# OSU-Nowlab/MPI4DL

Hardware: NVIDIA H100
Metric: images/sec (device-timed, max over ranks) AmoebaNet-D 8192^2 hot path (spatial-stage conv/pool fwd+bwd) (higher is better)
Workload: dtype bf16

## Files before the change

### include/spconv.h

```cpp
#ifndef SPCONV_H_
#define SPCONV_H_

#include <stddef.h>
#include <stdint.h>

#ifdef __cplusplus
extern "C" {
#endif

#define SPC_VERSION 101

enum { SPC_OK = 0, SPC_EINVAL = -1, SPC_ECUDA = -2, SPC_EUNSUPPORTED = -3, SPC_ENOMEM = -4 };
enum { SPC_F32 = 0, SPC_BF16 = 1 };
enum { SPC_POOL_MAX = 0, SPC_POOL_AVG = 1 };
enum {
  SPC_ALGO_AUTO = 0, SPC_ALGO_DIRECT = 1, SPC_ALGO_TCGEN05 = 2, SPC_ALGO_TF32 = 3, SPC_ALGO_TF32_ALL = 4,
  SPC_ALGO_TF32_STRIDED = 5
};

typedef struct {
  int32_t N, C, H, W;
  int32_t K, R, S;
  int32_t stride_h, stride_w;
  int32_t pad_h, pad_w;
// ... 11 lines not shown
typedef struct {
  const void* strip[9];
} spc_halo;

int         spc_version(void);
const char* spc_last_error(void);
int         spc_device_info(int device, int* sm_count, int* cc);
long long   spc_launch_count(int reset);
void        spc_reload_env(void);

int spc_conv2d_fwd(const spc_conv_desc* d, const void* x, const spc_halo* halo, const void* w,
                   const void* bias, void* y, void* workspace, size_t workspace_bytes,
                   void* stream);

int spc_conv2d_fwd_interior(const spc_conv_desc* d, const void* x, const void* w, const void* bias,
                            void* y, void* workspace, size_t workspace_bytes, void* stream);
int spc_conv2d_fwd_boundary(const spc_conv_desc* d, const void* x, const spc_halo* halo,
                            const void* w, const void* bias, void* y, void* stream);

int spc_conv2d_dgrad(const spc_conv_desc* d, const void* dy, const void* w, void* dx,
                     void* workspace, size_t workspace_bytes, void* stream);

int spc_conv2d_wgrad(const spc_conv_desc* d, const void* x, const spc_halo* halo, const void* dy,
                     float* dw, float* db, int accumulate, void* workspace,
                     size_t workspace_bytes, void* stream);

size_t spc_conv_workspace_bytes(const spc_conv_desc* d, int op );
int    spc_conv_uses_tcgen05(const spc_conv_desc* d, int op);
void   spc_conv_out_shape(const spc_conv_desc* d, int* Ho, int* Wo);

int spc_pool2d_fwd(const spc_pool_desc* d, const void* x, const spc_halo* halo, void* y, void* stream);
int spc_pool2d_bwd(const spc_pool_desc* d, const void* x, const spc_halo* halo, const void* dy,
                   void* dx, void* stream);

size_t spc_bn_workspace_bytes(int N, int C, long long HW);
int spc_bn_stats(int N, int C, long long HW, int dtype, const void* y, float* mean, float* var, void* workspace,
                 size_t workspace_bytes, void* stream);
int spc_bn_apply(int N, int C, long long HW, int dtype, const void* y, const float* mean, const float* rstd,
                 const float* gamma, const float* beta, int relu, void* z, void* stream);
int spc_bn_bwd_reduce(int N, int C, long long HW, int dtype, const void* dz, const void* y, const float* mean,
                      const float* rstd, const float* gamma, const float* beta, int relu, float* dsum,
                      float* dsumx, void* workspace, size_t workspace_bytes, void* stream);
int spc_bn_bwd_apply(int N, int C, long long HW, int dtype, const void* dz, const void* y, const float* mean,
                     const float* rstd, const float* gamma, const float* beta, int relu, const float* dsum,
                     const float* dsumx, void* dy, void* stream);

int spc_halo_pack(int N, int C, int H, int W, int halo_h, int halo_w, int dtype, const void* x,
                  void* const send[9], void* stream);
int spc_halo_pad(int N, int C, int H, int W, int halo_h, int halo_w, int dtype, const void* x,
                 const spc_halo* halo, void* y, void* stream);
int spc_halo_crop(int N, int C, int H, int W, int halo_h, int halo_w, int dtype, const void* dy,
                  void* dx, void* stream);

typedef struct spc_mailbox spc_mailbox;
#define SPC_IPC_HANDLE_BYTES 64
int   spc_mailbox_create(spc_mailbox** out, size_t bytes, int nflags);
void  spc_mailbox_destroy(spc_mailbox* mb);
void* spc_mailbox_data(spc_mailbox* mb);
int   spc_mailbox_export(spc_mailbox* mb, unsigned char handle[SPC_IPC_HANDLE_BYTES]);
int   spc_mailbox_open(spc_mailbox** out, const unsigned char handle[SPC_IPC_HANDLE_BYTES],
                       size_t bytes, int nflags);
int spc_halo_post(int N, int C, int H, int W, int halo_h, int halo_w, int dtype, const void* x,
                  void* const send[9], spc_mailbox* self, spc_mailbox* const peers[9],
                  const int ack_idx[9], uint32_t ack_seq, const int arrival_idx[9], uint32_t seq,
                  void* stream);
int spc_halo_collect(void* const dst[9], const void* const src[9], const size_t bytes[9],
// ... 29 lines not shown
```

### mpi4dl_b200/_lib.py

```python
import ctypes as C
import os

HERE = os.path.dirname(os.path.abspath(__file__))
LIB_PATH = os.path.join(HERE, "libspconv.so")

SPC_F32, SPC_BF16 = 0, 1
SPC_POOL_MAX, SPC_POOL_AVG = 0, 1
SPC_ALGO_AUTO, SPC_ALGO_DIRECT, SPC_ALGO_TCGEN05, SPC_ALGO_TF32, SPC_ALGO_TF32_ALL, SPC_ALGO_TF32_STRIDED = 0, 1, 2, 3, 4, 5
IPC_HANDLE_BYTES = 64


class ConvDesc(C.Structure):
    _fields_ = [(n, C.c_int32) for n in
                ("N", "C", "H", "W", "K", "R", "S", "stride_h", "stride_w", "pad_h", "pad_w", "dtype", "algo")]


class PoolDesc(C.Structure):
    _fields_ = [(n, C.c_int32) for n in ("N", "C", "H", "W", "k", "stride", "pad", "mode", "dtype")]


class Halo(C.Structure):
    _fields_ = [("strip", C.c_void_p * 9)]


_P = C.c_void_p
SYMBOLS = [
    ("spc_version", C.c_int, []),
    ("spc_last_error", C.c_char_p, []),
    ("spc_device_info", C.c_int, [C.c_int, C.POINTER(C.c_int), C.POINTER(C.c_int)]),
    ("spc_launch_count", C.c_longlong, [C.c_int]),
    ("spc_reload_env", None, []),
    ("spc_conv2d_fwd", C.c_int, [C.POINTER(ConvDesc), _P, C.POINTER(Halo), _P, _P, _P, _P, C.c_size_t, _P]),
    ("spc_conv2d_fwd_interior", C.c_int, [C.POINTER(ConvDesc), _P, _P, _P, _P, _P, C.c_size_t, _P]),
    ("spc_conv2d_fwd_boundary", C.c_int, [C.POINTER(ConvDesc), _P, C.POINTER(Halo), _P, _P, _P, _P]),
    ("spc_conv2d_dgrad", C.c_int, [C.POINTER(ConvDesc), _P, _P, _P, _P, C.c_size_t, _P]),
    ("spc_conv2d_wgrad", C.c_int, [C.POINTER(ConvDesc), _P, C.POINTER(Halo), _P, _P, _P, C.c_int, _P, C.c_size_t, _P]),
    ("spc_conv_workspace_bytes", C.c_size_t, [C.POINTER(ConvDesc), C.c_int]),
    ("spc_conv_uses_tcgen05", C.c_int, [C.POINTER(ConvDesc), C.c_int]),
    ("spc_conv_out_shape", None, [C.POINTER(ConvDesc), C.POINTER(C.c_int), C.POINTER(C.c_int)]),
    ("spc_pool2d_fwd", C.c_int, [C.POINTER(PoolDesc), _P, C.POINTER(Halo), _P, _P]),
    ("spc_pool2d_bwd", C.c_int, [C.POINTER(PoolDesc), _P, C.POINTER(Halo), _P, _P, _P]),
    ("spc_bn_workspace_bytes", C.c_size_t, [C.c_int, C.c_int, C.c_longlong]),
    ("spc_bn_stats", C.c_int, [C.c_int, C.c_int, C.c_longlong, C.c_int, _P, _P, _P, _P, C.c_size_t, _P]),
    ("spc_bn_apply", C.c_int, [C.c_int, C.c_int, C.c_longlong, C.c_int, _P, _P, _P, _P, _P, C.c_int, _P, _P]),
    ("spc_bn_bwd_reduce", C.c_int, [C.c_int, C.c_int, C.c_longlong, C.c_int, _P, _P, _P, _P, _P, _P, C.c_int, _P, _P, _P,
                                    C.c_size_t, _P]),
    ("spc_bn_bwd_apply", C.c_int, [C.c_int, C.c_int, C.c_longlong, C.c_int, _P, _P, _P, _P, _P, _P, C.c_int, _P, _P, _P, _P]),
    ("spc_halo_pack", C.c_int, [C.c_int] * 7 + [_P, C.POINTER(_P * 9), _P]),
    ("spc_halo_pad", C.c_int, [C.c_int] * 7 + [_P, C.POINTER(Halo), _P, _P]),
    ("spc_halo_crop", C.c_int, [C.c_int] * 7 + [_P, _P, _P]),
    ("spc_mailbox_create", C.c_int, [C.POINTER(_P), C.c_size_t, C.c_int]),
    ("spc_mailbox_destroy", None, [_P]),
    ("spc_mailbox_data", _P, [_P]),
    ("spc_mailbox_export", C.c_int, [_P, C.c_char_p]),
    ("spc_mailbox_open", C.c_int, [C.POINTER(_P), C.c_char_p, C.c_size_t, C.c_int]),
    ("spc_halo_post", C.c_int, [C.c_int] * 7 + [_P, C.POINTER(_P * 9), _P, C.POINTER(_P * 9), C.POINTER(C.c_int * 9),
                                C.c_uint32, C.POINTER(C.c_int * 9), C.c_uint32, _P]),
    ("spc_halo_collect", C.c_int, [C.POINTER(_P * 9), C.POINTER(_P * 9), C.POINTER(C.c_size_t * 9), _P, C.POINTER(_P * 9),
                                   C.POINTER(C.c_int * 9), C.c_uint32, C.POINTER(C.c_int * 9), _P]),
    ("spc_halo_post_auto", C.c_int, [C.c_int] * 7 + [_P, C.POINTER(_P * 9), C.c_size_t, _P, C.POINTER(_P * 9),
                                     C.POINTER(C.c_int * 9), C.POINTER(C.c_int * 9), C.c_int, C.c_int, _P]),
    ("spc_halo_collect_auto", C.c_int, [C.POINTER(_P * 9), C.POINTER(_P * 9), C.POINTER(C.c_size_t * 9), C.c_size_t, _P,
                                        C.POINTER(_P * 9), C.POINTER(C.c_int * 9), C.POINTER(C.c_int * 9), C.c_int, C.c_int,
                                        _P]),
    ("spc_conv2d_dgrad_halo", C.c_int, [C.POINTER(ConvDesc), _P, _P, C.POINTER(_P * 9), _P]),
    ("spc_pool2d_bwd_halo", C.c_int, [C.POINTER(PoolDesc), _P, C.POINTER(Halo), _P, C.POINTER(_P * 9), _P]),
    ("spc_halo_ring", C.c_int, [C.c_int] * 7 + [_P, C.POINTER(_P * 9), _P]),
    ("spc_halo_accumulate", C.c_int, [C.c_int] * 7 + [_P, C.POINTER(_P * 9), _P]),
    ("spc_halo_post_strips_auto", C.c_int, [C.POINTER(_P * 9), C.POINTER(C.c_size_t * 9), C.POINTER(_P * 9), C.c_size_t,
                                            _P, C.POINTER(_P * 9), C.POINTER(C.c_int * 9), C.POINTER(C.c_int * 9),
                                            C.c_int, C.c_int, _P]),
    ("spc_mailbox_signal", C.c_int, [_P, C.c_int, C.c_uint32, _P]),
    ("spc_mailbox_wait", C.c_int, [_P, C.c_int, C.c_uint32, _P]),
]
# ... 46 lines not shown
```

### mpi4dl_b200/build.py

```python
import os
import subprocess
import sys

HERE = os.path.dirname(os.path.abspath(__file__))
CSRC = os.path.join(HERE, "csrc")
LIB = os.path.join(HERE, "libspconv.so")
SOURCES = ["api.cu", "conv_direct.cu", "pool.cu", "halo.cu", "gemm_tc.cu", "conv_tap.cu", "wgrad_tap.cu", "bnrelu.cu",
           "halo_grad.cu", "gemm_tf32.cu", "conv_tap_tf32.cu", "conv_tap_s2_tf32.cu",
           "gemm_px.cu"]
NVCC_FLAGS = [
    "-O3", "-std=c++17", "-gencode", "arch=compute_90a,code=sm_90a", "-lineinfo",
    "-Xcompiler", "-fPIC", "--expt-relaxed-constexpr",
]


def _stale(target, deps):
    if not os.path.exists(target):
        return True
    t = os.path.getmtime(target)
    return any(os.path.getmtime(d) > t for d in deps)


def build_lib(force=False, verbose=False):
    nvcc = os.environ.get("NVCC", "/usr/local/cuda/bin/nvcc")
    hdrs = [os.path.join(CSRC, f) for f in os.listdir(CSRC) if f.endswith((".cuh", ".h"))]
    hdrs.append(os.path.join(HERE, "..", "include", "spconv.h"))
    objs = []
    procs = []
    for s in SOURCES:
        src = os.path.join(CSRC, s)
        obj = os.path.join(CSRC, s.replace(".cu", ".o"))
        objs.append(obj)
        if force or _stale(obj, [src] + hdrs):
            cmd = [nvcc] + NVCC_FLAGS + (["-Xptxas", "-v"] if verbose else []) + ["-c", src, "-o", obj]
            procs.append((s, subprocess.Popen(cmd, stdout=subprocess.PIPE, stderr=subprocess.STDOUT, text=True)))
    for s, p in procs:
        out, _ = p.communicate()
        if p.returncode != 0:
            sys.stderr.write(out)
            raise RuntimeError("nvcc failed on %s" % s)
        if verbose:
            sys.stderr.write(out)
# ... 9 lines not shown
```

### mpi4dl_b200/csrc/common.cuh

```cuda
#pragma once
#include <cuda_bf16.h>
#include <cuda_runtime.h>
#include <stdint.h>
#include <stdio.h>

#include "../../include/spconv.h"

namespace spc {

void set_error(const char* fmt, ...);
void count_launch(int n = 1);

#define SPC_CHECK_CUDA(expr)                                                              \
  do {                                                                                    \
    cudaError_t _e = (expr);                                                              \
    if (_e != cudaSuccess) {                                                              \
      spc::set_error("%s:%d CUDA error %s: %s", __FILE__, __LINE__, #expr,                \
                     cudaGetErrorString(_e));                                             \
      return SPC_ECUDA;                                                                   \
    }                                                                                     \
  } while (0)

#define SPC_REQUIRE(cond, ...)                                                            \
  do {                                                                                    \
    if (!(cond)) {                                                                        \
      spc::set_error(__VA_ARGS__);                                                        \
      return SPC_EINVAL;                                                                  \
    }                                                                                     \
  } while (0)

template <typename T> __device__ __forceinline__ float to_f32(T v);
template <> __device__ __forceinline__ float to_f32<float>(float v) { return v; }
template <> __device__ __forceinline__ float to_f32<__nv_bfloat16>(__nv_bfloat16 v) { return __bfloat162float(v); }
template <typename T> __device__ __forceinline__ T from_f32(float v);
template <> __device__ __forceinline__ float from_f32<float>(float v) { return v; }
template <> __device__ __forceinline__ __nv_bfloat16 from_f32<__nv_bfloat16>(float v) { return __float2bfloat16_rn(v); }

__device__ __forceinline__ bool pool_max_takes(float v, float m) { return (v > m) | (v != v); }
__device__ __forceinline__ float pool_max(float m, float v) {
  float r;
  asm("max.NaN.f32 %0, %1, %2;" : "=f"(r) : "f"(m), "f"(v));
  return r;
}

struct TileView {
  const void* x;
  const void* strip[9];
  int N, C, H, W;
  int hh, hw;
};

template <typename T>
__device__ __forceinline__ float tile_load(const TileView& v, int n, int c, int h, int w) {
  const bool hin = (unsigned)h < (unsigned)v.H;
  const bool win = (unsigned)w < (unsigned)v.W;
  if (hin && win) {
    if (v.x == nullptr) return 0.f;
    return to_f32<T>(reinterpret_cast<const T*>(v.x)[(((size_t)n * v.C + c) * v.H + h) * v.W + w]);
  }
  const int dr = h < 0 ? 0 : (hin ? 1 : 2);
  const int dc = w < 0 ? 0 : (win ? 1 : 2);
  const T* s = reinterpret_cast<const T*>(v.strip[dr * 3 + dc]);
  if (s == nullptr) return 0.f;
  const int sh = (dr == 1) ? v.H : v.hh;
  const int sw = (dc == 1) ? v.W : v.hw;
  const int y = (dr == 0) ? h + v.hh : (dr == 2 ? h - v.H : h);
  const int xx = (dc == 0) ? w + v.hw : (dc == 2 ? w - v.W : w);
  if ((unsigned)y >= (unsigned)sh || (unsigned)xx >= (unsigned)sw) return 0.f;
  return to_f32<T>(s[(((size_t)n * v.C + c) * sh + y) * sw + xx]);
}

template <typename T>
__device__ __forceinline__ const T* tile_ptr(const TileView& v, int n, int c, int h, int w) {
  const bool hin = (unsigned)h < (unsigned)v.H;
  const bool win = (unsigned)w < (unsigned)v.W;
// ... 104 lines not shown
```

### mpi4dl_b200/csrc/gemm_tc.cu

```cuda
#include <stdlib.h>

#include "common.cuh"
#include "tc_common.cuh"

namespace spc {

using namespace tc;

bool tap_v2_supported(int M, int Cin, int R, int S, int H, int W, int N, int stride);
int run_conv_tap_v2(const __nv_bfloat16* wp, int Mpad, int Cpad, const __nv_bfloat16* x, const __nv_bfloat16* bias,
                    __nv_bfloat16* y, int M, int Cin, int R, int S, int ph, int H, int W, int N, cudaStream_t st);

bool wgrad_tap_supported(int K, int C, int R, int S, int H, int W, int stride);
int run_wgrad_tap(const __nv_bfloat16* x, const __nv_bfloat16* dy, float* dw, int K, int C, int N, int H, int W, int R, int S,
                  cudaStream_t st);

int run_pw_px(int NT, const CUtensorMap& tw, const CUtensorMap& tx, const CUtensorMap& ty, int M, int Cin, int N, int P,
              int x5, int y5, const __nv_bfloat16* bias, int sms, cudaStream_t st);

namespace {

constexpr int TC_THREADS = 384;
constexpr int BK = 64;
constexpr int A_BLK_BYTES = 128 * BK * 2;
// ... 806 lines not shown
    const __nv_bfloat16* t0 = t + ((n * 4 + 2 * a) * C + c) * plane + (size_t)oy * Wo + v * 8;
    const uint4 e = __ldg(reinterpret_cast<const uint4*>(t0));
    const uint4 o = __ldg(reinterpret_cast<const uint4*>(t0 + (size_t)C * plane));
    uint4 lo, hi;
    lo.x = __byte_perm(e.x, o.x, 0x5410); lo.y = __byte_perm(e.x, o.x, 0x7632);
    lo.z = __byte_perm(e.y, o.y, 0x5410); lo.w = __byte_perm(e.y, o.y, 0x7632);
    hi.x = __byte_perm(e.z, o.z, 0x5410); hi.y = __byte_perm(e.z, o.z, 0x7632);
    hi.z = __byte_perm(e.w, o.w, 0x5410); hi.w = __byte_perm(e.w, o.w, 0x7632);
    uint4* d = reinterpret_cast<uint4*>(dx + ((nc * 2 * Ho) + 2 * oy + a) * (size_t)(2 * Wo) + v * 16);
    d[0] = lo; d[1] = hi;
  }
}

__global__ void subsample2_kernel(const __nv_bfloat16* __restrict__ x, __nv_bfloat16* __restrict__ y, size_t planes,
                                  int H, int W) {
  const int Ho = H / 2, Wo = W / 2, wv = Wo / 8;
  const size_t total = planes * Ho * wv;
  for (size_t i = (size_t)blockIdx.x * blockDim.x + threadIdx.x; i < total; i += (size_t)gridDim.x * blockDim.x) {
    const int v = (int)(i % wv);
    const int oy = (int)((i / wv) % Ho);
    const size_t pl = i / ((size_t)wv * Ho);
    const uint4* src = reinterpret_cast<const uint4*>(x + (pl * H + 2 * oy) * W + v * 16);
    const uint4 a = __ldg(src), b = __ldg(src + 1);
    uint4 o;
    o.x = __byte_perm(a.x, a.y, 0x5410);
    o.y = __byte_perm(a.z, a.w, 0x5410);
    o.z = __byte_perm(b.x, b.y, 0x5410);
    o.w = __byte_perm(b.z, b.w, 0x5410);
    *reinterpret_cast<uint4*>(y + (pl * Ho + oy) * Wo + v * 8) = o;
  }
}
__global__ void upsample2_zero_kernel(const __nv_bfloat16* __restrict__ g, __nv_bfloat16* __restrict__ dx,
                                      size_t planes, int H, int W) {
  const int Ho = H / 2, Wo = W / 2, wv = Wo / 8;
  const size_t total = planes * Ho * wv;
  const uint4 z = make_uint4(0, 0, 0, 0);
  for (size_t i = (size_t)blockIdx.x * blockDim.x + threadIdx.x; i < total; i += (size_t)gridDim.x * blockDim.x) {
    const int v = (int)(i % wv);
    const int oy = (int)((i / wv) % Ho);
    const size_t pl = i / ((size_t)wv * Ho);
    const uint4 a = __ldg(reinterpret_cast<const uint4*>(g + (pl * Ho + oy) * Wo + v * 8));
    uint4 lo, hi;
    lo.x = a.x & 0xFFFFu; lo.y = a.x >> 16; lo.z = a.y & 0xFFFFu; lo.w = a.y >> 16;
    hi.x = a.z & 0xFFFFu; hi.y = a.z >> 16; hi.z = a.w & 0xFFFFu; hi.w = a.w >> 16;
    uint4* d0 = reinterpret_cast<uint4*>(dx + (pl * H + 2 * oy) * W + v * 16);
    uint4* d1 = reinterpret_cast<uint4*>(dx + (pl * H + 2 * oy + 1) * W + v * 16);
    d0[0] = lo; d0[1] = hi; d1[0] = z; d1[1] = z;
  }
}
int launch_resample(bool up, const void* src, void* dst, size_t planes, int H, int W, cudaStream_t st) {
  const size_t total = planes * (H / 2) * (W / 16);
  size_t blocks = (total + 255) / 256;
  if (blocks > 132 * 32) blocks = 132 * 32;
  if (up)
    upsample2_zero_kernel<<<(int)blocks, 256, 0, st>>>((const __nv_bfloat16*)src, (__nv_bfloat16*)dst, planes, H, W);
  else
    subsample2_kernel<<<(int)blocks, 256, 0, st>>>((const __nv_bfloat16*)src, (__nv_bfloat16*)dst, planes, H, W);
  count_launch();
  SPC_CHECK_CUDA(cudaGetLastError());
  return SPC_OK;
}

__global__ void shift_copies_kernel(const __nv_bfloat16* __restrict__ x, __nv_bfloat16* __restrict__ xs,
                                    size_t planes, int H, int W, int S, int pw, int cs) {
  const int Wv = W / cs;
  const int wv = Wv / 8;
  const size_t rows = planes * H;
  const size_t total = rows * wv * S;
  for (size_t i = (size_t)blockIdx.x * blockDim.x + threadIdx.x; i < total; i += (size_t)gridDim.x * blockDim.x) {
    const int v = (int)(i % wv);
    const size_t row = (i / wv) % rows;
    const int sidx = (int)(i / ((size_t)wv * rows));
    const __nv_bfloat16* src = x + row * W;
    const int w0 = v * 8 * cs + sidx - pw;
    __nv_bfloat16 e[8];
#pragma unroll
    for (int j = 0; j < 8; ++j) {
      const int w = w0 + j * cs;
      e[j] = ((unsigned)w < (unsigned)W) ? src[w] : __float2bfloat16(0.f);
    }
    *reinterpret_cast<uint4*>(xs + ((size_t)sidx * rows + row) * Wv + v * 8) = *reinterpret_cast<const uint4*>(e);
  }
}
template <int S, int PW>
// ... 298 lines not shown
```

### mpi4dl_b200/csrc/pool.cu

```cuda
#include <cuda.h>

#include "common.cuh"
#include "tc_common.cuh"

namespace spc {
namespace {

struct PoolParams {
  TileView in;
  const void* dy;
  void* out;
  int k, stride, pad, mode, Ho, Wo;
};

template <typename T>
__global__ void pool_fwd_kernel(const PoolParams p) {
  const size_t total = (size_t)p.in.N * p.in.C * p.Ho * p.Wo;
  const float inv = 1.f / (float)(p.k * p.k);
  for (size_t i = (size_t)blockIdx.x * blockDim.x + threadIdx.x; i < total; i += (size_t)gridDim.x * blockDim.x) {
    const int ox = (int)(i % p.Wo);
    const int oy = (int)((i / p.Wo) % p.Ho);
    const size_t nc = i / ((size_t)p.Wo * p.Ho);
    const int c = (int)(nc % p.in.C), n = (int)(nc / p.in.C);
    const int h0 = oy * p.stride - p.pad, w0 = ox * p.stride - p.pad;
    float r = (p.mode == SPC_POOL_MAX) ? -INFINITY : 0.f;
    for (int a = 0; a < p.k; ++a)
      for (int b = 0; b < p.k; ++b) {
        const float v = tile_load<T>(p.in, n, c, h0 + a, w0 + b);
        r = (p.mode == SPC_POOL_MAX) ? pool_max(r, v) : r + v;
      }
    if (p.mode == SPC_POOL_AVG) r *= inv;
    reinterpret_cast<T*>(p.out)[i] = from_f32<T>(r);
  }
}

template <typename T, int NEL>
__device__ __forceinline__ void load_vec(const T* __restrict__ src, float (&dst)[NEL]) {
  constexpr int NV = NEL * sizeof(T) / 16;
  uint4 raw[NV];
#pragma unroll
  for (int q = 0; q < NV; ++q) raw[q] = __ldg(reinterpret_cast<const uint4*>(src) + q);
  const T* e = reinterpret_cast<const T*>(raw);
#pragma unroll
  for (int j = 0; j < NEL; ++j) dst[j] = to_f32<T>(e[j]);
}
template <typename T, int NEL>
__device__ __forceinline__ void store_vec(T* __restrict__ dst, const float (&src)[NEL]) {
  constexpr int NV = NEL * sizeof(T) / 16;
  uint4 raw[NV];
  T* e = reinterpret_cast<T*>(raw);
#pragma unroll
  for (int j = 0; j < NEL; ++j) e[j] = from_f32<T>(src[j]);
#pragma unroll
  for (int q = 0; q < NV; ++q) reinterpret_cast<uint4*>(dst)[q] = raw[q];
}

template <typename T, int VEC, int K, int STRIDE>
__global__ void __launch_bounds__(256)
pool_fwd_vec_kernel(const PoolParams p) {
  constexpr int PAD = (K - 1) / 2;
  constexpr int SPAN = (VEC - 1) * STRIDE + K;
  constexpr int IN_VEC = VEC * STRIDE;
  const int wv = p.Wo / VEC;
  const size_t total = (size_t)p.in.N * p.in.C * p.Ho * wv;
  const float inv = 1.f / (float)(K * K);
  const T* x = reinterpret_cast<const T*>(p.in.x);
  for (size_t i = (size_t)blockIdx.x * blockDim.x + threadIdx.x; i < total; i += (size_t)gridDim.x * blockDim.x) {
    const int vx = (int)(i % wv);
    const int oy = (int)((i / wv) % p.Ho);
    const size_t nc = i / ((size_t)wv * p.Ho);
    const int c = (int)(nc % p.in.C), n = (int)(nc / p.in.C);
    const int ox0 = vx * VEC;
    const int w0 = ox0 * STRIDE - PAD;
    const int h0 = oy * STRIDE - PAD;
    float acc[VEC];
#pragma unroll
    for (int j = 0; j < VEC; ++j) acc[j] = (p.mode == SPC_POOL_MAX) ? -INFINITY : 0.f;
#pragma unroll
    for (int a = 0; a < K; ++a) {
      const int h = h0 + a;
      float row[SPAN];
      const bool row_in = (unsigned)h < (unsigned)p.in.H;
      if (row_in) {
        const T* src = x + (((size_t)n * p.in.C + c) * p.in.H + h) * p.in.W + (w0 + PAD);
        if constexpr (sizeof(T) * IN_VEC % 16 == 0) {
          constexpr int NV = sizeof(T) * IN_VEC / 16;
          uint4 raw[NV];
// ... 308 lines not shown
    const int hp = h + p.pad, wp = w + p.pad;
    int oy_lo = (hp - p.k + 1 + p.stride - 1);
    oy_lo = oy_lo < 0 ? 0 : oy_lo / p.stride;
    int ox_lo = (wp - p.k + 1 + p.stride - 1);
    ox_lo = ox_lo < 0 ? 0 : ox_lo / p.stride;
    const int oy_hi = min(p.Ho - 1, hp / p.stride), ox_hi = min(p.Wo - 1, wp / p.stride);
    float g = 0.f;
    const T* dyp = dy + nc * (size_t)p.Ho * p.Wo;
    if (p.mode == SPC_POOL_AVG) {
      for (int oy = oy_lo; oy <= oy_hi; ++oy)
        for (int ox = ox_lo; ox <= ox_hi; ++ox) g += to_f32<T>(dyp[(size_t)oy * p.Wo + ox]);
      g *= inv;
    } else {
      for (int oy = oy_lo; oy <= oy_hi; ++oy)
        for (int ox = ox_lo; ox <= ox_hi; ++ox) {
          const int h0 = oy * p.stride - p.pad, w0 = ox * p.stride - p.pad;
          float best = -INFINITY;
          int bi = 0;
          for (int a = 0; a < p.k; ++a)
            for (int b = 0; b < p.k; ++b) {
              const float v = tile_load<T>(p.in, n, c, h0 + a, w0 + b);
              if (pool_max_takes(v, best)) { best = v; bi = a * p.k + b; }
            }
          if (bi == (h - h0) * p.k + (w - w0)) g += to_f32<T>(dyp[(size_t)oy * p.Wo + ox]);
        }
    }
    reinterpret_cast<T*>(p.out)[i] = from_f32<T>(g);
  }
}

template <typename T, int MODE>
__global__ void __launch_bounds__(256)
pool_bwd_s2_vec_kernel(const PoolParams p) {
  constexpr int V = 8;
  const int H = p.in.H, W = p.in.W, Ho = p.Ho, Wo = p.Wo;
  const int wv = Wo / V;
  const size_t total = (size_t)p.in.N * p.in.C * Ho * wv;
  const T* dy = reinterpret_cast<const T*>(p.dy);
  const T* x = reinterpret_cast<const T*>(p.in.x);
  T* dx = reinterpret_cast<T*>(p.out);
  for (size_t i = (size_t)blockIdx.x * blockDim.x + threadIdx.x; i < total; i += (size_t)gridDim.x * blockDim.x) {
    const int vx = (int)(i % wv);
    const int oy = (int)((i / wv) % Ho);
    const size_t nc = i / ((size_t)wv * Ho);
    const int ox0 = vx * V;
    const T* g0 = dy + (nc * Ho + oy) * Wo + ox0;
    float g[V + 1], gn[V + 1];
    {
      float gv[V];
      load_vec<T, V>(g0, gv);
#pragma unroll
      for (int j = 0; j < V; ++j) g[j] = gv[j];
    }
    float o0[2 * V], o1[2 * V];
    if (MODE == SPC_POOL_AVG) {
      const bool has_r = ox0 + V < Wo, has_d = oy + 1 < Ho;
      g[V] = has_r ? to_f32<T>(g0[V]) : 0.f;
      if (has_d) {
        float gv[V];
        load_vec<T, V>(g0 + Wo, gv);
#pragma unroll
        for (int j = 0; j < V; ++j) gn[j] = gv[j];
        gn[V] = has_r ? to_f32<T>(g0[Wo + V]) : 0.f;
      } else {
#pragma unroll
        for (int j = 0; j <= V; ++j) gn[j] = 0.f;
      }
      const float inv = 1.f / 9.f;
#pragma unroll
      for (int j = 0; j < V; ++j) {
        o0[2 * j] = g[j] * inv;
        o0[2 * j + 1] = (g[j] + g[j + 1]) * inv;
        o1[2 * j] = (g[j] + gn[j]) * inv;
        o1[2 * j + 1] = (g[j] + g[j + 1] + gn[j] + gn[j + 1]) * inv;
      }
    } else {
      const T* x0 = x + (nc * H + 2 * oy) * W + 2 * ox0;
      float r0[2 * V], r1[2 * V];
      load_vec<T, 2 * V>(x0, r0);
      load_vec<T, 2 * V>(x0 + W, r1);
#pragma unroll
      for (int j = 0; j < V; ++j) {
        const float a = r0[2 * j], b = r0[2 * j + 1];
        const float c = r1[2 * j], d = r1[2 * j + 1];
        int best = 0;
        float m = a;
        if (b > m) { m = b; best = 1; }
        if (c > m) { m = c; best = 2; }
        if (d > m) { m = d; best = 3; }
        if (isnan(a) || isnan(b) || isnan(c) || isnan(d)) best = isnan(d) ? 3 : isnan(c) ? 2 : isnan(b) ? 1 : 0;
        o0[2 * j] = best == 0 ? g[j] : 0.f;
        o0[2 * j + 1] = best == 1 ? g[j] : 0.f;
        o1[2 * j] = best == 2 ? g[j] : 0.f;
        o1[2 * j + 1] = best == 3 ? g[j] : 0.f;
      }
    }
    T* d0 = dx + (nc * H + 2 * oy) * W + 2 * ox0;
    store_vec<T, 2 * V>(d0, o0);
    store_vec<T, 2 * V>(d0 + W, o1);
  }
}

template <typename T>
int run_fwd(const PoolParams& p, cudaStream_t st) {
  const size_t total = (size_t)p.in.N * p.in.C * p.Ho * p.Wo;
  if (total == 0) return SPC_OK;
  constexpr int VEC = 16 / sizeof(T);
  const bool aligned = ((uintptr_t)p.in.x % 16 == 0) && ((uintptr_t)p.out % 16 == 0);
  const bool vec_ok = aligned && p.Wo % VEC == 0 && p.in.W % (VEC * p.stride) == 0 &&
                      p.in.W == p.Wo * p.stride;
  const size_t vtotal = total / VEC;
  const int blocks = (int)((vtotal + 255) / 256 > 132 * 32 ? 132 * 32 : (vtotal + 255) / 256);
  if (vec_ok && p.k == 3 && p.stride == 1) {
    return launch_pool3_tma<T>(p, st);
  } else if (vec_ok && p.k == 3 && p.stride == 2) {
    pool3_fwd_kernel<T, VEC, 2><<<blocks, 256, 0, st>>>(p);
  } else if (vec_ok && p.k == 2 && p.stride == 2) {
    pool_fwd_vec_kernel<T, VEC, 2, 2><<<blocks, 256, 0, st>>>(p);
  } else {
    const int b2 = (int)((total + 255) / 256 > 132 * 32 ? 132 * 32 : (total + 255) / 256);
    pool_fwd_kernel<T><<<b2, 256, 0, st>>>(p);
  }
  spc::count_launch();
  SPC_CHECK_CUDA(cudaGetLastError());
  return SPC_OK;
}

template <typename T>
int run_bwd(const PoolParams& p, cudaStream_t st) {
  const size_t total = (size_t)p.in.N * p.in.C * p.in.H * p.in.W;
  if (total == 0) return SPC_OK;
  const int blocks = (int)((total + 255) / 256 > 132 * 32 ? 132 * 32 : (total + 255) / 256);
  const bool aligned = ((uintptr_t)p.in.x % 16 == 0) && ((uintptr_t)p.out % 16 == 0) && ((uintptr_t)p.dy % 16 == 0);
  const bool even = aligned && p.in.W % 16 == 0 && p.in.H % 2 == 0 && p.in.W == 2 * p.Wo && p.in.H == 2 * p.Ho;
  if (p.mode == SPC_POOL_AVG && p.k == 3 && p.stride == 1 && aligned && p.in.W % (16 / sizeof(T)) == 0) {
    PoolParams q = p;
    q.in = make_view(p.dy, nullptr, p.in.N, p.in.C, p.Ho, p.Wo, 1, 1);
    q.dy = nullptr;
    return launch_pool3_tma<T>(q, st);
  } else if (even && p.mode == SPC_POOL_AVG && p.k == 3 && p.stride == 2) {
    const size_t vt = total / 32;
    const int b2 = (int)((vt + 255) / 256 > 132 * 32 ? 132 * 32 : (vt + 255) / 256);
    pool_bwd_s2_vec_kernel<T, SPC_POOL_AVG><<<b2, 256, 0, st>>>(p);
  } else if (even && p.mode == SPC_POOL_MAX && p.k == 2 && p.stride == 2) {
    const size_t vt = total / 32;
    const int b2 = (int)((vt + 255) / 256 > 132 * 32 ? 132 * 32 : (vt + 255) / 256);
    pool_bwd_s2_vec_kernel<T, SPC_POOL_MAX><<<b2, 256, 0, st>>>(p);
  } else {
    pool_bwd_kernel<T><<<blocks, 256, 0, st>>>(p);
  }
  spc::count_launch();
  SPC_CHECK_CUDA(cudaGetLastError());
  return SPC_OK;
}

int fill(PoolParams& p, const spc_pool_desc* d, const void* x, const spc_halo* halo) {
  SPC_REQUIRE(d && x, "pool: null descriptor or input");
  SPC_REQUIRE(d->k >= 1 && d->stride >= 1 && d->pad == (d->k - 1) / 2,
              "pool: pad must equal floor((k-1)/2) (reference spatial.py:1457-1464), got k=%d pad=%d", d->k, d->pad);
  SPC_REQUIRE(d->mode == SPC_POOL_MAX || d->mode == SPC_POOL_AVG, "pool: bad mode %d", d->mode);
  SPC_REQUIRE(d->dtype == SPC_F32 || d->dtype == SPC_BF16, "pool: bad dtype %d", d->dtype);
  p.in = make_view(x, halo, d->N, d->C, d->H, d->W, d->pad, d->pad);
  p.k = d->k; p.stride = d->stride; p.pad = d->pad; p.mode = d->mode;
  p.Ho = (d->H + 2 * d->pad - d->k) / d->stride + 1;
  p.Wo = (d->W + 2 * d->pad - d->k) / d->stride + 1;
  return SPC_OK;
}

}
}

extern "C" int spc_pool2d_fwd(const spc_pool_desc* d, const void* x, const spc_halo* halo, void* y, void* stream) {
  spc::PoolParams p{};
  int rc = spc::fill(p, d, x, halo);
  if (rc) return rc;
  p.out = y; p.dy = nullptr;
  return d->dtype == SPC_BF16 ? spc::run_fwd<__nv_bfloat16>(p, (cudaStream_t)stream)
                              : spc::run_fwd<float>(p, (cudaStream_t)stream);
// ... 12 lines not shown
```

### mpi4dl_b200/torchgems/spatial.py

```python
import ctypes as C
import math
import os
import threading
import warnings

import torch
import torch.distributed as dist
import torch.nn as nn

from .. import _lib
from . import halo_transport

_DIRS = [(-1, -1), (-1, 0), (-1, 1), (0, -1), (0, 0), (0, 1), (1, -1), (1, 0), (1, 1)]


def _stream():
    return C.c_void_p(torch.cuda.current_stream().cuda_stream)


def _require_cuda(t, who):
    if not t.is_cuda:
        raise RuntimeError(
            "%s: input must be a CUDA tensor -- the spatial conv path runs only on libspconv "
            "(sm_90a); there is no CPU fallback" % who)
# ... 415 lines not shown

    def __init__(self, local_rank, spatial_size, num_spatial_parts, halo_len, padding_mode="zeros",
                 slice_method="square"):
        super(halo_exchange_layer, self).__init__()
        self._init_topology(local_rank, spatial_size, num_spatial_parts, slice_method)
        self.halo_len = halo_len
        self.get_neighbours()
        self.rank_neighbours = [-1] * 9
        if self.neighbours is not None:
            self.get_neighbours_rank()
        self.set_tags()
        self.exact_backward = halo_transport.exact_backward_default()

    def forward(self, tensor):
        _require_cuda(tensor, "halo_exchange_layer")
        x = tensor.contiguous()
        with torch.no_grad():
            strips = self._exchange(x, self.halo_len, self.halo_len) if self.halo_len > 0 else [None] * 9
        tail = (self,) if self.exact_backward and any(s is not None for s in strips) else ()
        return _HaloPadFn.apply(x, self.halo_len, *strips, *tail)


class _PoolFn(torch.autograd.Function):
    @staticmethod
    def forward(ctx, x, desc_args, *strips):
        L = _lib.lib()
        d = _lib.PoolDesc(*desc_args)
        ctx.n_tail = len(strips)
        ctx.layer = strips[9] if len(strips) > 9 else None
        strips = strips[:9]
        Ho = (d.H + 2 * d.pad - d.k) // d.stride + 1
        Wo = (d.W + 2 * d.pad - d.k) // d.stride + 1
        y = torch.empty((d.N, d.C, Ho, Wo), dtype=x.dtype, device=x.device)
        halo = _lib.make_halo(strips)
        _lib.check(L.spc_pool2d_fwd(C.byref(d), _ptr(x), C.byref(halo), _ptr(y), _stream()), "spc_pool2d_fwd")
        ctx.desc_args = desc_args
        ctx.save_for_backward(x, *[s for s in strips if s is not None])
        ctx.strip_mask = [s is not None for s in strips]
        return y

    @staticmethod
    def backward(ctx, gy):
        L = _lib.lib()
        saved = ctx.saved_tensors
        x = saved[0]
        it = iter(saved[1:])
        strips = [next(it) if m else None for m in ctx.strip_mask]
        d = _lib.PoolDesc(*ctx.desc_args)
        gy = gy.contiguous()
        halo = _lib.make_halo(strips)
        exact = ctx.layer is not None and ctx.needs_input_grad[0]
        if exact:
            grads = _alloc_strip_grads(ctx.layer.neighbours, d.N, d.C, d.H, d.W, d.pad, d.pad, x.device)
            _lib.check(L.spc_pool2d_bwd_halo(C.byref(d), _ptr(x), C.byref(halo), _ptr(gy), C.byref(_strip_ptrs(grads)),
                                             _stream()), "spc_pool2d_bwd_halo")
            recv, ready = _reverse_begin(ctx.layer, grads, x.shape, d.pad, d.pad)
        dx = torch.empty_like(x)
        _lib.check(L.spc_pool2d_bwd(C.byref(d), _ptr(x), C.byref(halo), _ptr(gy), _ptr(dx), _stream()),
                   "spc_pool2d_bwd")
        if exact:
            _reverse_finish(recv, ready, dx, d.pad, d.pad)
        return (dx, None) + (None,) * ctx.n_tail


class Pool(nn.Module, _SpatialTopology):

    def __init__(self, local_rank, spatial_size, num_spatial_parts, kernel_size, stride, padding,
                 slice_method="square", dilation=1, return_indices=False, count_include_pad=True,
                 divisor_override=None, ceil_mode=False, operation=None):
        super(Pool, self).__init__()
        assert dilation == 1, "dilation > 1, Not Supported"
        assert return_indices == False, "return_indices == True, not supported"
        assert ceil_mode == False, "ceil model == True, not supported"
        assert operation != None, "operation is none"
        if isinstance(kernel_size, int):
            kernel_size = (kernel_size, kernel_size)
# ... 88 lines not shown
```

Baseline: 3.362.

## Store 2-bit argmax codes for 2x2 max-pool backward instead of saving input

Adds a fused 2x2 stride-2 max-pool forward kernel that also writes a packed 2-bit argmax code per output. Backward then scatters the gradient using only the codes and no longer re-reads the input, and the saved activation shrinks from the full input to a small code buffer. Also narrows the per-thread vector width in the upsample and s2 pool backward kernels to raise thread count. The risk is that the code path skips the halo strips, so it is only valid for pad 0, and that narrower vectors issue more memory instructions.

Result: faster. 3.481, median of 6 (+3.5%).

```diff
diff --git a/include/spconv.h b/include/spconv.h
--- a/include/spconv.h
+++ b/include/spconv.h
@@ -67,6 +67,9 @@
 int spc_pool2d_fwd(const spc_pool_desc* d, const void* x, const spc_halo* halo, void* y, void* stream);
 int spc_pool2d_bwd(const spc_pool_desc* d, const void* x, const spc_halo* halo, const void* dy,
                    void* dx, void* stream);
+size_t spc_pool_code_bytes(const spc_pool_desc* d);
+int spc_pool2d_fwd_code(const spc_pool_desc* d, const void* x, void* y, void* code, void* stream);
+int spc_pool2d_bwd_code(const spc_pool_desc* d, const void* code, const void* dy, void* dx, void* stream);
 
 size_t spc_bn_workspace_bytes(int N, int C, long long HW);
 int spc_bn_stats(int N, int C, long long HW, int dtype, const void* y, float* mean, float* var, void* workspace,
diff --git a/mpi4dl_b200/_lib.py b/mpi4dl_b200/_lib.py
--- a/mpi4dl_b200/_lib.py
+++ b/mpi4dl_b200/_lib.py
@@ -40,6 +40,9 @@
     ("spc_conv_out_shape", None, [C.POINTER(ConvDesc), C.POINTER(C.c_int), C.POINTER(C.c_int)]),
     ("spc_pool2d_fwd", C.c_int, [C.POINTER(PoolDesc), _P, C.POINTER(Halo), _P, _P]),
     ("spc_pool2d_bwd", C.c_int, [C.POINTER(PoolDesc), _P, C.POINTER(Halo), _P, _P, _P]),
+    ("spc_pool_code_bytes", C.c_size_t, [C.POINTER(PoolDesc)]),
+    ("spc_pool2d_fwd_code", C.c_int, [C.POINTER(PoolDesc), _P, _P, _P, _P]),
+    ("spc_pool2d_bwd_code", C.c_int, [C.POINTER(PoolDesc), _P, _P, _P, _P]),
     ("spc_bn_workspace_bytes", C.c_size_t, [C.c_int, C.c_int, C.c_longlong]),
     ("spc_bn_stats", C.c_int, [C.c_int, C.c_int, C.c_longlong, C.c_int, _P, _P, _P, _P, C.c_size_t, _P]),
     ("spc_bn_apply", C.c_int, [C.c_int, C.c_int, C.c_longlong, C.c_int, _P, _P, _P, _P, _P, C.c_int, _P, _P]),
diff --git a/mpi4dl_b200/build.py b/mpi4dl_b200/build.py
--- a/mpi4dl_b200/build.py
+++ b/mpi4dl_b200/build.py
@@ -7,7 +7,7 @@
 LIB = os.path.join(HERE, "libspconv.so")
 SOURCES = ["api.cu", "conv_direct.cu", "pool.cu", "halo.cu", "gemm_tc.cu", "conv_tap.cu", "wgrad_tap.cu", "bnrelu.cu",
            "halo_grad.cu", "gemm_tf32.cu", "conv_tap_tf32.cu", "conv_tap_s2_tf32.cu",
-           "gemm_px.cu"]
+           "gemm_px.cu", "pool_code.cu"]
 NVCC_FLAGS = [
     "-O3", "-std=c++17", "-gencode", "arch=compute_90a,code=sm_90a", "-lineinfo",
     "-Xcompiler", "-fPIC", "--expt-relaxed-constexpr",
diff --git a/mpi4dl_b200/csrc/common.cuh b/mpi4dl_b200/csrc/common.cuh
--- a/mpi4dl_b200/csrc/common.cuh
+++ b/mpi4dl_b200/csrc/common.cuh
@@ -41,6 +41,44 @@
   float r;
   asm("max.NaN.f32 %0, %1, %2;" : "=f"(r) : "f"(m), "f"(v));
   return r;
+}
+__device__ __forceinline__ int pool_argmax4(float a, float b, float c, float d) {
+  int best = 0;
+  float m = a;
+  if (b > m) { m = b; best = 1; }
+  if (c > m) { m = c; best = 2; }
+  if (d > m) { m = d; best = 3; }
+  if (isnan(a) || isnan(b) || isnan(c) || isnan(d)) best = isnan(d) ? 3 : isnan(c) ? 2 : isnan(b) ? 1 : 0;
+  return best;
+}
+
+template <typename T, int NEL>
+__device__ __forceinline__ void load_vec(const T* __restrict__ src, float (&dst)[NEL]) {
+  static_assert(NEL * sizeof(T) % 16 == 0 || NEL * sizeof(T) == 8, "load_vec: 8 bytes or a multiple of 16");
+  if constexpr (NEL * sizeof(T) == 8) {
+    const uint2 raw = __ldg(reinterpret_cast<const uint2*>(src));
+    const T* e = reinterpret_cast<const T*>(&raw);
+#pragma unroll
+    for (int j = 0; j < NEL; ++j) dst[j] = to_f32<T>(e[j]);
+  } else {
+    constexpr int NV = NEL * sizeof(T) / 16;
+    uint4 raw[NV];
+#pragma unroll
+    for (int q = 0; q < NV; ++q) raw[q] = __ldg(reinterpret_cast<const uint4*>(src) + q);
+    const T* e = reinterpret_cast<const T*>(raw);
+#pragma unroll
+    for (int j = 0; j < NEL; ++j) dst[j] = to_f32<T>(e[j]);
+  }
+}
+template <typename T, int NEL>
+__device__ __forceinline__ void store_vec(T* __restrict__ dst, const float (&src)[NEL]) {
+  constexpr int NV = NEL * sizeof(T) / 16;
+  uint4 raw[NV];
+  T* e = reinterpret_cast<T*>(raw);
+#pragma unroll
+  for (int j = 0; j < NEL; ++j) e[j] = from_f32<T>(src[j]);
+#pragma unroll
+  for (int q = 0; q < NV; ++q) reinterpret_cast<uint4*>(dst)[q] = raw[q];
 }
 
 struct TileView {
diff --git a/mpi4dl_b200/csrc/gemm_tc.cu b/mpi4dl_b200/csrc/gemm_tc.cu
--- a/mpi4dl_b200/csrc/gemm_tc.cu
+++ b/mpi4dl_b200/csrc/gemm_tc.cu
@@ -862,24 +862,23 @@
 }
 __global__ void upsample2_zero_kernel(const __nv_bfloat16* __restrict__ g, __nv_bfloat16* __restrict__ dx,
                                       size_t planes, int H, int W) {
-  const int Ho = H / 2, Wo = W / 2, wv = Wo / 8;
+  const int Ho = H / 2, Wo = W / 2, wv = Wo / 4;
   const size_t total = planes * Ho * wv;
   const uint4 z = make_uint4(0, 0, 0, 0);
   for (size_t i = (size_t)blockIdx.x * blockDim.x + threadIdx.x; i < total; i += (size_t)gridDim.x * blockDim.x) {
     const int v = (int)(i % wv);
     const int oy = (int)((i / wv) % Ho);
     const size_t pl = i / ((size_t)wv * Ho);
-    const uint4 a = __ldg(reinterpret_cast<const uint4*>(g + (pl * Ho + oy) * Wo + v * 8));
-    uint4 lo, hi;
-    lo.x = a.x & 0xFFFFu; lo.y = a.x >> 16; lo.z = a.y & 0xFFFFu; lo.w = a.y >> 16;
-    hi.x = a.z & 0xFFFFu; hi.y = a.z >> 16; hi.z = a.w & 0xFFFFu; hi.w = a.w >> 16;
-    uint4* d0 = reinterpret_cast<uint4*>(dx + (pl * H + 2 * oy) * W + v * 16);
-    uint4* d1 = reinterpret_cast<uint4*>(dx + (pl * H + 2 * oy + 1) * W + v * 16);
-    d0[0] = lo; d0[1] = hi; d1[0] = z; d1[1] = z;
+    const uint2 a = __ldg(reinterpret_cast<const uint2*>(g + (pl * Ho + oy) * Wo + v * 4));
+    uint4 o;
+    o.x = a.x & 0xFFFFu; o.y = a.x >> 16; o.z = a.y & 0xFFFFu; o.w = a.y >> 16;
+    __nv_bfloat16* d0 = dx + (pl * H + 2 * oy) * W + v * 8;
+    *reinterpret_cast<uint4*>(d0) = o;
+    *reinterpret_cast<uint4*>(d0 + W) = z;
   }
 }
 int launch_resample(bool up, const void* src, void* dst, size_t planes, int H, int W, cudaStream_t st) {
-  const size_t total = planes * (H / 2) * (W / 16);
+  const size_t total = planes * (H / 2) * (W / (up ? 8 : 16));
   size_t blocks = (total + 255) / 256;
   if (blocks > 132 * 32) blocks = 132 * 32;
   if (up)
diff --git a/mpi4dl_b200/csrc/pool.cu b/mpi4dl_b200/csrc/pool.cu
--- a/mpi4dl_b200/csrc/pool.cu
+++ b/mpi4dl_b200/csrc/pool.cu
@@ -32,27 +32,6 @@
     if (p.mode == SPC_POOL_AVG) r *= inv;
     reinterpret_cast<T*>(p.out)[i] = from_f32<T>(r);
   }
-}
-
-template <typename T, int NEL>
-__device__ __forceinline__ void load_vec(const T* __restrict__ src, float (&dst)[NEL]) {
-  constexpr int NV = NEL * sizeof(T) / 16;
-  uint4 raw[NV];
-#pragma unroll
-  for (int q = 0; q < NV; ++q) raw[q] = __ldg(reinterpret_cast<const uint4*>(src) + q);
-  const T* e = reinterpret_cast<const T*>(raw);
-#pragma unroll
-  for (int j = 0; j < NEL; ++j) dst[j] = to_f32<T>(e[j]);
-}
-template <typename T, int NEL>
-__device__ __forceinline__ void store_vec(T* __restrict__ dst, const float (&src)[NEL]) {
-  constexpr int NV = NEL * sizeof(T) / 16;
-  uint4 raw[NV];
-  T* e = reinterpret_cast<T*>(raw);
-#pragma unroll
-  for (int j = 0; j < NEL; ++j) e[j] = from_f32<T>(src[j]);
-#pragma unroll
-  for (int q = 0; q < NV; ++q) reinterpret_cast<uint4*>(dst)[q] = raw[q];
 }
 
 template <typename T, int VEC, int K, int STRIDE>
@@ -427,7 +406,7 @@
 template <typename T, int MODE>
 __global__ void __launch_bounds__(256)
 pool_bwd_s2_vec_kernel(const PoolParams p) {
-  constexpr int V = 8;
+  constexpr int V = 8 / sizeof(T);
   const int H = p.in.H, W = p.in.W, Ho = p.Ho, Wo = p.Wo;
   const int wv = Wo / V;
   const size_t total = (size_t)p.in.N * p.in.C * Ho * wv;
@@ -478,12 +457,7 @@
       for (int j = 0; j < V; ++j) {
         const float a = r0[2 * j], b = r0[2 * j + 1];
         const float c = r1[2 * j], d = r1[2 * j + 1];
-        int best = 0;
-        float m = a;
-        if (b > m) { m = b; best = 1; }
-        if (c > m) { m = c; best = 2; }
-        if (d > m) { m = d; best = 3; }
-        if (isnan(a) || isnan(b) || isnan(c) || isnan(d)) best = isnan(d) ? 3 : isnan(c) ? 2 : isnan(b) ? 1 : 0;
+        const int best = pool_argmax4(a, b, c, d);
         o0[2 * j] = best == 0 ? g[j] : 0.f;
         o0[2 * j + 1] = best == 1 ? g[j] : 0.f;
         o1[2 * j] = best == 2 ? g[j] : 0.f;
@@ -534,11 +508,11 @@
     q.dy = nullptr;
     return launch_pool3_tma<T>(q, st);
   } else if (even && p.mode == SPC_POOL_AVG && p.k == 3 && p.stride == 2) {
-    const size_t vt = total / 32;
+    const size_t vt = total / (32 / sizeof(T));
     const int b2 = (int)((vt + 255) / 256 > 132 * 32 ? 132 * 32 : (vt + 255) / 256);
     pool_bwd_s2_vec_kernel<T, SPC_POOL_AVG><<<b2, 256, 0, st>>>(p);
   } else if (even && p.mode == SPC_POOL_MAX && p.k == 2 && p.stride == 2) {
-    const size_t vt = total / 32;
+    const size_t vt = total / (32 / sizeof(T));
     const int b2 = (int)((vt + 255) / 256 > 132 * 32 ? 132 * 32 : (vt + 255) / 256);
     pool_bwd_s2_vec_kernel<T, SPC_POOL_MAX><<<b2, 256, 0, st>>>(p);
   } else {
diff --git a/mpi4dl_b200/csrc/pool_code.cu b/mpi4dl_b200/csrc/pool_code.cu
--- /dev/null
+++ b/mpi4dl_b200/csrc/pool_code.cu
@@ -0,0 +1,135 @@
+#include "common.cuh"
+
+namespace spc {
+namespace {
+
+struct CodeParams {
+  const void* x;
+  const void* dy;
+  void* out;
+  uint16_t* code;
+  const uint16_t* code_in;
+  size_t planes;
+  int H, W, Ho, Wo;
+};
+
+constexpr int CV = 8;
+
+template <typename T>
+__global__ void __launch_bounds__(256)
+pool2_max_code_fwd_kernel(const CodeParams p) {
+  const int wv = p.Wo / CV;
+  const size_t total = p.planes * p.Ho * wv;
+  const T* x = reinterpret_cast<const T*>(p.x);
+  T* y = reinterpret_cast<T*>(p.out);
+  for (size_t i = (size_t)blockIdx.x * blockDim.x + threadIdx.x; i < total; i += (size_t)gridDim.x * blockDim.x) {
+    const int vx = (int)(i % wv);
+    const size_t row = i / wv;
+    const int oy = (int)(row % p.Ho);
+    const size_t nc = row / p.Ho;
+    const T* x0 = x + (nc * p.H + 2 * oy) * p.W + 2 * vx * CV;
+    float r0[2 * CV], r1[2 * CV], o[CV];
+    load_vec<T, 2 * CV>(x0, r0);
+    load_vec<T, 2 * CV>(x0 + p.W, r1);
+    uint32_t code = 0;
+#pragma unroll
+    for (int j = 0; j < CV; ++j) {
+      const float a = r0[2 * j], b = r0[2 * j + 1];
+      const float c = r1[2 * j], d = r1[2 * j + 1];
+      o[j] = pool_max(pool_max(pool_max(pool_max(-INFINITY, a), b), c), d);
+      code |= (uint32_t)pool_argmax4(a, b, c, d) << (2 * j);
+    }
+    store_vec<T, CV>(y + row * p.Wo + vx * CV, o);
+    p.code[i] = (uint16_t)code;
+  }
+}
+
+template <typename T>
+__global__ void __launch_bounds__(256)
+pool2_max_code_bwd_kernel(const CodeParams p) {
+  constexpr int BV = 8 / sizeof(T);
+  const int wv = p.Wo / BV;
+  const size_t total = p.planes * p.Ho * wv;
+  const T* dy = reinterpret_cast<const T*>(p.dy);
+  T* dx = reinterpret_cast<T*>(p.out);
+  for (size_t i = (size_t)blockIdx.x * blockDim.x + threadIdx.x; i < total; i += (size_t)gridDim.x * blockDim.x) {
+    const int vx = (int)(i % wv);
+    const size_t row = i / wv;
+    const int oy = (int)(row % p.Ho);
+    const size_t nc = row / p.Ho;
+    const uint2 graw = __ldg(reinterpret_cast<const uint2*>(dy + row * p.Wo + vx * BV));
+    const T* ge = reinterpret_cast<const T*>(&graw);
+    const uint32_t code = (uint32_t)__ldg(p.code_in + i * BV / CV) >> (2 * (i * BV % CV));
+    float o0[2 * BV], o1[2 * BV];
+#pragma unroll
+    for (int j = 0; j < BV; ++j) {
+      const float g = to_f32<T>(ge[j]);
+      const uint32_t best = (code >> (2 * j)) & 3u;
+      o0[2 * j] = best == 0 ? g : 0.f;
+      o0[2 * j + 1] = best == 1 ? g : 0.f;
+      o1[2 * j] = best == 2 ? g : 0.f;
+      o1[2 * j + 1] = best == 3 ? g : 0.f;
+    }
+    T* d0 = dx + (nc * p.H + 2 * oy) * p.W + 2 * vx * BV;
+    store_vec<T, 2 * BV>(d0, o0);
+    store_vec<T, 2 * BV>(d0 + p.W, o1);
+  }
+}
+
+bool eligible(const spc_pool_desc* d) {
+  return d && d->N > 0 && d->C > 0 && d->H > 0 && d->W > 0 && d->mode == SPC_POOL_MAX && d->k == 2 &&
+         d->stride == 2 && d->pad == 0 && (d->dtype == SPC_F32 || d->dtype == SPC_BF16) && d->H % 2 == 0 &&
+         d->W % 16 == 0;
+}
+
+int fill(CodeParams& p, const spc_pool_desc* d) {
+  SPC_REQUIRE(eligible(d), "pool code: needs max pooling, k=2, stride 2, pad 0, bf16 or fp32, even H and W %% 16 == 0");
+  p.planes = (size_t)d->N * d->C;
+  p.H = d->H; p.W = d->W; p.Ho = d->H / 2; p.Wo = d->W / 2;
+  return SPC_OK;
+}
+
+template <typename T>
+int launch(const CodeParams& p, bool fwd, cudaStream_t st) {
+  const size_t vt = p.planes * p.Ho * (p.Wo / (fwd ? CV : 8 / (int)sizeof(T)));
+  const int blocks = (int)((vt + 255) / 256 > 132 * 32 ? 132 * 32 : (vt + 255) / 256);
+  if (fwd)
+    pool2_max_code_fwd_kernel<T><<<blocks, 256, 0, st>>>(p);
+  else
+    pool2_max_code_bwd_kernel<T><<<blocks, 256, 0, st>>>(p);
+  count_launch();
+  SPC_CHECK_CUDA(cudaGetLastError());
+  return SPC_OK;
+}
+
+bool aligned16(const void* q) { return q != nullptr && (uintptr_t)q % 16 == 0; }
+
+}
+}
+
+extern "C" size_t spc_pool_code_bytes(const spc_pool_desc* d) {
+  if (!spc::eligible(d)) return 0;
+  return (size_t)d->N * d->C * (d->H / 2) * (d->W / 2) / 4;
+}
+
+extern "C" int spc_pool2d_fwd_code(const spc_pool_desc* d, const void* x, void* y, void* code, void* stream) {
+  spc::CodeParams p{};
+  int rc = spc::fill(p, d);
+  if (rc) return rc;
+  SPC_REQUIRE(spc::aligned16(x) && spc::aligned16(y) && code && (uintptr_t)code % 2 == 0,
+              "pool code: x and y must be 16-byte aligned and code 2-byte aligned");
+  p.x = x; p.out = y; p.code = static_cast<uint16_t*>(code);
+  return d->dtype == SPC_BF16 ? spc::launch<__nv_bfloat16>(p, true, (cudaStream_t)stream)
+                              : spc::launch<float>(p, true, (cudaStream_t)stream);
+}
+
+extern "C" int spc_pool2d_bwd_code(const spc_pool_desc* d, const void* code, const void* dy, void* dx, void* stream) {
+  spc::CodeParams p{};
+  int rc = spc::fill(p, d);
+  if (rc) return rc;
+  SPC_REQUIRE(spc::aligned16(dy) && spc::aligned16(dx) && code && (uintptr_t)code % 2 == 0,
+              "pool code: dy and dx must be 16-byte aligned and code 2-byte aligned");
+  p.dy = dy; p.out = dx; p.code_in = static_cast<const uint16_t*>(code);
+  return d->dtype == SPC_BF16 ? spc::launch<__nv_bfloat16>(p, false, (cudaStream_t)stream)
+                              : spc::launch<float>(p, false, (cudaStream_t)stream);
+}
diff --git a/mpi4dl_b200/torchgems/spatial.py b/mpi4dl_b200/torchgems/spatial.py
--- a/mpi4dl_b200/torchgems/spatial.py
+++ b/mpi4dl_b200/torchgems/spatial.py
@@ -471,9 +471,16 @@
         Ho = (d.H + 2 * d.pad - d.k) // d.stride + 1
         Wo = (d.W + 2 * d.pad - d.k) // d.stride + 1
         y = torch.empty((d.N, d.C, Ho, Wo), dtype=x.dtype, device=x.device)
+        ctx.desc_args = desc_args
+        code_bytes = L.spc_pool_code_bytes(C.byref(d)) if x.data_ptr() % 16 == 0 else 0
+        ctx.use_code = code_bytes > 0
+        if ctx.use_code:
+            code = torch.empty(code_bytes, dtype=torch.uint8, device=x.device)
+            _lib.check(L.spc_pool2d_fwd_code(C.byref(d), _ptr(x), _ptr(y), _ptr(code), _stream()), "spc_pool2d_fwd_code")
+            ctx.save_for_backward(code)
+            return y
         halo = _lib.make_halo(strips)
         _lib.check(L.spc_pool2d_fwd(C.byref(d), _ptr(x), C.byref(halo), _ptr(y), _stream()), "spc_pool2d_fwd")
-        ctx.desc_args = desc_args
         ctx.save_for_backward(x, *[s for s in strips if s is not None])
         ctx.strip_mask = [s is not None for s in strips]
         return y
@@ -481,6 +488,15 @@
     @staticmethod
     def backward(ctx, gy):
         L = _lib.lib()
+        if ctx.use_code:
+            code, = ctx.saved_tensors
+            d = _lib.PoolDesc(*ctx.desc_args)
+            gy = gy.contiguous()
+            if gy.data_ptr() % 16:
+                gy = gy.clone()
+            dx = torch.empty((d.N, d.C, d.H, d.W), dtype=gy.dtype, device=gy.device)
+            _lib.check(L.spc_pool2d_bwd_code(C.byref(d), _ptr(code), _ptr(gy), _ptr(dx), _stream()), "spc_pool2d_bwd_code")
+            return (dx, None) + (None,) * ctx.n_tail
         saved = ctx.saved_tensors
         x = saved[0]
         it = iter(saved[1:])
```
